# Shulk97/JPEG_detection_Resnet_SSD

Measured on AMD Instinct MI355X. Metric: images/sec (train) ResNet50-DCT-SSD300, higher is better.
Workload: dtype f32; 1 GPU; SSD300 ResNet50-DCT 'deconv' archi, 32 images/GPU, 300x300 JPEG-DCT inputs (Y 38x38x64 + chroma 19x19), fwd+loss+bwd+SGD(+RCCL all-reduce); batch and encoded targets resident in HBM: host->device upload, target encoding and the per-step loss read-back of fit_generator are outside the timed region (DESIGN.md section 6 has those rates); archi=deconv, global_batch=32, parallelism=dp1

## Files before the change

include/dj_hip.h:

```cpp
#ifndef DJ_HIP_H
#define DJ_HIP_H
#include <stddef.h>
#include <stdint.h>

#ifdef __cplusplus
extern "C" {
#endif

const char* dj_last_error(void);
#define DJ_ABI_VERSION 3
int dj_abi_version(void);

#define DJ_F32 0
#define DJ_F16 1
#define DJ_BF16 2

typedef struct dj_conv2d_desc {
  int batch;
  int in_h, in_w, in_c;
  int out_h, out_w, out_c;
  int kernel_h, kernel_w;
  int stride_h, stride_w;
  int dilation_h, dilation_w;
  int pad_top, pad_left;
// ... 25 lines not shown
int dj_conv2d_nhwc_dgrad_relumask(const dj_conv2d_desc* d, const float* dy, const float* w, const float* bias, float* dx,
                                  int beta, const float* mask_x, int ld_mask, void* stream);

int dj_conv2d_fwd_addrelu_supported(const dj_conv2d_desc* d);
int dj_conv2d_nhwc_fwd_addrelu(const dj_conv2d_desc* d, const float* x, const float* w, const float* bias, float* y,
                               const float* pro_scale, const float* pro_shift, const float* res, int ld_res,
                               const float* res_scale, const float* res_shift, float* sum_out, int ld_sum, int relu,
                               float* stats, void* stream);
int dj_conv2d_nhwc_fwd_addrelu_ws(const dj_conv2d_desc* d, const float* x, const float* w, const float* bias, float* y,
                                  const float* pro_scale, const float* pro_shift, const float* res, int ld_res,
                                  const float* res_scale, const float* res_shift, float* sum_out, int ld_sum, int relu,
                                  float* stats, float* workspace, long workspace_floats, void* stream);

#define DJ_BN_ACC_REPLICAS 16
typedef struct dj_bn_train {
  double* acc;
  unsigned* ticket;
  const float* gamma;
  const float* beta;
  float* moving_mean;
  float* moving_var;
  float* scale;
  float* shift;
  float* save_mean;
  float* save_invstd;
  float eps, momentum;
} dj_bn_train;
int dj_conv2d_nhwc_fwd_bn(const dj_conv2d_desc* d, const float* x, const float* w, const float* bias, float* y,
                          const float* pro_scale, const float* pro_shift, int pro_relu, const float* res, int ld_res,
                          const float* res_scale, const float* res_shift, float* sum_out, int ld_sum,
                          const dj_bn_train* bn, void* stream);

void dj_set_fast_path(int enable);

int dj_set_compute_mode(int mode);
int dj_set_thread_compute_mode(int mode);
int dj_get_compute_mode(void);

int dj_conv2d_tune_configs(void);
int dj_conv2d_tune_set(int dir, const dj_conv2d_desc* d, int cfg, int splits);
int dj_conv2d_default_config(int dir, const dj_conv2d_desc* d, int* cfg, int* splits);

int dj_conv2d_nhwc_wgrad(const dj_conv2d_desc* d, const float* x, const float* dy, float* dw,
                         const float* pro_scale, const float* pro_shift, int pro_relu, int dw_zeroed, void* stream);

int dj_conv2d_nhwc_fwd_t(const dj_conv2d_desc* d, const void* x, int dt_x, const void* w, int dt_w, const float* bias, void* y,
                         int dt_y, const float* pro_scale, const float* pro_shift, int pro_relu, int relu, float* stats,
                         const void* res, int ld_res, const float* res_scale, const float* res_shift, void* sum_out,
                         int ld_sum, int dt_sum, float* workspace, long workspace_floats, void* stream);
int dj_conv2d_nhwc_dgrad_t(const dj_conv2d_desc* d, const void* dy, int dt_dy, const void* w, int dt_w, const float* bias,
                           void* dx, int dt_dx, int beta, const void* z, int ld_z, int dt_z, const float* mean, const float* invstd,
                           const float* scale, const float* shift, float* partial, void* stream);
int dj_shadow_weights(const float* w, void* w16, void* wbf, long n, void* stream);
int dj_conv2d_nhwc_wgrad_t(const dj_conv2d_desc* d, const void* x, int dt_x, const void* dy, int dt_dy, float* dw,
                           const float* pro_scale, const float* pro_shift, int pro_relu, int dw_zeroed, void* stream);

int dj_reduce_rows(long rows);
int dj_colstats_partial(const float* x, long rows, int C, int ld, float* partial, void* stream);
int dj_colsum_partial(const float* dy, long rows, int C, int ld, float* partial, void* stream);
int dj_colreduce_finalize(const float* partial, int nrows, int C, int which, float* out, int beta, void* stream);
int dj_colsum_direct(const float* x, long rows, int C, int ld, float* out, int beta, void* stream);
#define DJ_COLSUM_PARTS 32
typedef struct dj_colsum_part {
  const float* x;
  float* out;
  long rows;
// ... 215 lines not shown
```

jpeg_detection_resnet_ssd_amd/_lib.py:

```python
import ctypes
import os
from ctypes import POINTER, Structure, c_char_p, c_double, c_float, c_int, c_long, c_void_p

_HERE = os.path.dirname(os.path.abspath(__file__))
LIB_PATH = os.environ.get("DJ_LIB_PATH") or os.path.join(_HERE, "csrc", "libdj_hip.so")


class DjError(RuntimeError):
    pass


class BnTrain(Structure):
    _fields_ = [("acc", c_void_p), ("ticket", c_void_p), ("gamma", c_void_p), ("beta", c_void_p),
                ("moving_mean", c_void_p), ("moving_var", c_void_p), ("scale", c_void_p), ("shift", c_void_p),
                ("save_mean", c_void_p), ("save_invstd", c_void_p), ("eps", c_float), ("momentum", c_float)]


class CopyPart(Structure):
    _fields_ = [("src", c_void_p), ("dst", c_void_p), ("ld_src", c_long), ("ld_dst", c_long), ("rows", c_long),
                ("cols", c_long), ("beta", c_int)]


class ColsumPart(Structure):
    _fields_ = [("x", c_void_p), ("out", c_void_p), ("rows", c_long), ("C", c_int), ("ld", c_int), ("beta", c_int)]
# ... 66 lines not shown
    "dj_conv2d_nhwc_fwd": (c_int, [POINTER(ConvDesc), FP, FP, FP, FP, FP, FP, c_int, c_int, FP, c_void_p]),
    "dj_conv2d_nhwc_fwd_ws": (c_int, [POINTER(ConvDesc), FP, FP, FP, FP, FP, FP, c_int, c_int, FP, FP, c_long, c_void_p]),
    "dj_conv2d_fwd_workspace_floats": (c_long, [POINTER(ConvDesc), c_int]),
    "dj_conv2d_nhwc_dgrad": (c_int, [POINTER(ConvDesc), FP, FP, FP, FP, c_int, c_void_p]),
    "dj_conv2d_nhwc_dgrad_bnbwd": (c_int, [POINTER(ConvDesc), FP, FP, FP, FP, c_int, FP, FP, FP, FP, FP, c_void_p]),
    "dj_conv2d_dgrad_relumask_supported": (c_int, [POINTER(ConvDesc)]),
    "dj_conv2d_nhwc_dgrad_relumask": (c_int, [POINTER(ConvDesc), FP, FP, FP, FP, c_int, FP, c_int, c_void_p]),
    "dj_conv2d_nhwc_wgrad": (c_int, [POINTER(ConvDesc), FP, FP, FP, FP, FP, c_int, c_int, c_void_p]),
    "dj_conv2d_nhwc_fwd_t": (c_int, [POINTER(ConvDesc), FP, c_int, FP, c_int, FP, FP, c_int, FP, FP, c_int, c_int, FP, FP, c_int, FP,
                                     FP, FP, c_int, c_int, FP, c_long, c_void_p]),
    "dj_conv2d_nhwc_dgrad_t": (c_int, [POINTER(ConvDesc), FP, c_int, FP, c_int, FP, FP, c_int, c_int, FP, c_int, c_int, FP, FP, FP,
                                       FP, FP, c_void_p]),
    "dj_shadow_weights": (c_int, [FP, FP, FP, c_long, c_void_p]),
    "dj_conv2d_nhwc_wgrad_t": (c_int, [POINTER(ConvDesc), FP, c_int, FP, c_int, FP, FP, FP, c_int, c_int, c_void_p]),
    "dj_affine_act_t": (c_int, [FP, c_int, c_int, FP, FP, FP, c_int, c_int, FP, FP, FP, c_int, c_int, c_long, c_int, c_int,
                                c_void_p]),
    "dj_bn_bwd_reduce_t": (c_int, [FP, c_int, c_int, FP, c_int, c_int, FP, c_int, c_int, FP, FP, FP, FP, c_int, c_long, c_int, FP,
                                   c_void_p]),
    "dj_bn_bwd_apply_t": (c_int, [FP, c_int, c_int, FP, c_int, c_int, FP, c_int, c_int, FP, FP, c_int, FP, FP, FP, FP, c_int,
                                  c_int, c_long, c_int, FP, c_int, c_int, c_int, c_void_p]),
    "dj_relu_bwd_t": (c_int, [FP, c_int, c_int, FP, c_int, c_int, FP, c_int, c_int, c_long, c_int, c_int, c_void_p]),
    "dj_copy2d_t": (c_int, [FP, c_int, c_long, FP, c_int, c_long, c_long, c_long, c_int, c_void_p]),
    "dj_conv2d_fwd_addrelu_supported": (c_int, [POINTER(ConvDesc)]),
    "dj_conv2d_nhwc_fwd_addrelu": (c_int, [POINTER(ConvDesc), FP, FP, FP, FP, FP, FP, FP, c_int, FP, FP, FP, c_int, c_int, FP,
                                           c_void_p]),
    "dj_conv2d_nhwc_fwd_addrelu_ws": (c_int, [POINTER(ConvDesc), FP, FP, FP, FP, FP, FP, FP, c_int, FP, FP, FP, c_int, c_int,
                                              FP, FP, c_long, c_void_p]),
    "dj_colsum_direct": (c_int, [FP, c_long, c_int, c_int, FP, c_int, c_void_p]),
    "dj_colsum_multi": (c_int, [POINTER(ColsumPart), c_int, c_void_p]),
    "dj_copy2d_multi": (c_int, [POINTER(CopyPart), c_int, c_void_p]),
    "dj_conv2d_nhwc_fwd_bn": (c_int, [POINTER(ConvDesc), FP, FP, FP, FP, FP, FP, c_int, FP, c_int, FP, FP, FP, c_int,
                                      POINTER(BnTrain), c_void_p]),
    "dj_set_fast_path": (None, [c_int]),
    "dj_set_compute_mode": (c_int, [c_int]),
    "dj_set_thread_compute_mode": (c_int, [c_int]),
    "dj_get_compute_mode": (c_int, []),
    "dj_conv2d_tune_configs": (c_int, []),
    "dj_conv2d_tune_set": (c_int, [c_int, POINTER(ConvDesc), c_int, c_int]),
    "dj_conv2d_default_config": (c_int, [c_int, POINTER(ConvDesc), POINTER(c_int), POINTER(c_int)]),
    "dj_reduce_rows": (c_int, [c_long]),
    "dj_colstats_partial": (c_int, [FP, c_long, c_int, c_int, FP, c_void_p]),
    "dj_colsum_partial": (c_int, [FP, c_long, c_int, c_int, FP, c_void_p]),
    "dj_colreduce_finalize": (c_int, [FP, c_int, c_int, c_int, FP, c_int, c_void_p]),
    "dj_bn_train_finalize": (c_int, [FP, c_int, c_long, FP, FP, FP, c_float, c_float, FP, FP, FP, FP, FP, FP, c_int,
                                     c_void_p]),
    "dj_bn_infer_coeffs": (c_int, [FP, FP, FP, FP, c_float, FP, FP, c_int, c_void_p]),
    "dj_affine_act": (c_int, [FP, c_int, FP, FP, FP, c_int, FP, FP, FP, c_int, c_long, c_int, c_int, c_void_p]),
    "dj_bn_bwd_reduce": (c_int, [FP, c_int, FP, c_int, FP, c_int, FP, FP, FP, FP, c_int, c_long, c_int, FP, c_void_p]),
    "dj_bn_bwd_finalize": (c_int, [FP, c_int, c_long, FP, FP, FP, FP, FP, FP, FP, FP, c_int, c_void_p]),
    "dj_bn_bwd_apply": (c_int, [FP, c_int, FP, c_int, FP, c_int, FP, FP, c_int, FP, FP, FP, FP, c_int, c_long, c_int,
                                FP, c_int, c_int, c_void_p]),
    "dj_relu_bwd": (c_int, [FP, c_int, FP, c_int, FP, c_int, c_long, c_int, c_int, c_void_p]),
    "dj_copy2d": (c_int, [FP, c_long, FP, c_long, c_long, c_long, c_int, c_void_p]),
    "dj_upsample2x": (c_int, [FP, c_int, FP, c_int, c_int, c_int, c_int, c_int, c_void_p]),
    "dj_l2norm_fwd": (c_int, [FP, c_int, FP, FP, c_int, FP, c_long, c_int, c_void_p]),
    "dj_l2norm_bwd": (c_int, [FP, c_int, FP, c_int, FP, FP, FP, c_int, FP, c_long, c_int, c_int, c_void_p]),
    "dj_maxpool2d_fwd": (c_int, [FP, FP] + [c_int] * 13 + [c_void_p, c_void_p]),
    "dj_maxpool2d_bwd": (c_int, [FP, FP, FP] + [c_int] * 14 + [c_void_p, c_void_p]),
    "dj_softmax_fwd": (c_int, [FP, FP, c_long, c_int, c_void_p]),
    "dj_softmax_bwd": (c_int, [FP, FP, c_long, FP, c_long, c_int, c_int, c_void_p]),
    "dj_ssd_loss_workspace_floats": (c_long, [c_long]),
    "dj_ssd_loss_fwd": (c_int, [FP, FP, c_long, c_int, c_int, c_int, c_float, FP, FP, c_void_p]),
    "dj_ssd_loss_bwd": (c_int, [FP, FP, c_long, c_int, c_float, c_float, FP, FP, FP, c_void_p]),
    "dj_categorical_crossentropy": (c_int, [FP, FP, c_long, c_int, c_float, FP, FP, FP, c_void_p]),
    "dj_sgd_momentum_update": (c_int, [FP, FP, FP, c_long, c_float, c_float, c_int, c_float, c_float, FP, c_void_p]),
    "dj_decode_detections_workspace_floats": (c_long, [c_int, c_int, c_int, c_int]),
# ... 73 lines not shown
```

jpeg_detection_resnet_ssd_amd/csrc/dj_conv.hip:

```cpp
#include "../../include/dj_hip.h"
#include "dj_conv_launch.h"
#include <string.h>
#include <map>
#include <mutex>
#include <atomic>
#include <array>
#include <algorithm>

static thread_local char g_err[512] = "";
void dj_set_error(const char* fmt, ...) {
  va_list ap;
  va_start(ap, fmt);
  vsnprintf(g_err, sizeof(g_err), fmt, ap);
  va_end(ap);
}
extern "C" const char* dj_last_error(void) { return g_err; }
extern "C" int dj_abi_version(void) { return DJ_ABI_VERSION; }

std::atomic<bool> g_dj_allow_fast{true};
extern "C" void dj_set_fast_path(int enable) { g_dj_allow_fast.store(enable != 0, std::memory_order_relaxed); }

static std::atomic<int> g_default_compute_mode{0};
static thread_local int tl_compute_mode = -1;
int dj_compute_mode() { return tl_compute_mode >= 0 ? tl_compute_mode : g_default_compute_mode.load(std::memory_order_relaxed); }
extern "C" int dj_set_compute_mode(int mode) {
  int prev = g_default_compute_mode.load(std::memory_order_relaxed);
  if (mode >= 0 && mode <= 5) g_default_compute_mode.store(mode, std::memory_order_relaxed);
  return prev;
}
extern "C" int dj_set_thread_compute_mode(int mode) {
  int prev = tl_compute_mode;
  if (mode >= -1 && mode <= 5) tl_compute_mode = mode;
  return prev;
}
extern "C" int dj_get_compute_mode(void) { return dj_compute_mode(); }

extern template int dj_launch_cfg<0, 0>(int, const DjIgemmParams&, int, hipStream_t);
extern template int dj_launch_cfg<0, 1>(int, const DjIgemmParams&, int, hipStream_t);
extern template int dj_launch_cfg<1, 1>(int, const DjIgemmParams&, int, hipStream_t);
extern template int dj_launch_cfg<2, 0>(int, const DjIgemmParams&, int, hipStream_t);

static int choose_cfg(long M, long N, long K, bool allow_split, int* splits_out) {
  int bn;
  if (N > 96) {
    long pad128 = (long)dj_cdiv(N, 128) * 128, pad64 = (long)dj_cdiv(N, 64) * 64;
    bn = (pad64 < pad128) ? 64 : 128;
  } else if (N > 32 && (long)dj_cdiv(N, 64) * 64 <= (long)dj_cdiv(N, 32) * 32) {
    bn = 64;
  } else {
    bn = 32;
  }
  int cfg;
  auto tiles = [&](int bm, int b_n) { return (long)dj_cdiv(M, bm) * dj_cdiv(N, b_n); };
// ... 791 lines not shown
```

jpeg_detection_resnet_ssd_amd/csrc/dj_conv_launch.h:

```cpp
#pragma once
#include "../../include/dj_hip.h"
#include "dj_igemm.h"
#include "dj_igemm_fast.h"
#include <stdlib.h>
#include <atomic>

struct TileCfg {
  int bm, bn;
};
static const TileCfg kCfgs[] = {{128, 128}, {128, 64}, {64, 64}, {128, 32}, {128, 128}, {128, 64}, {64, 64}, {64, 64}, {128, 64}, {128, 128}, {128, 64}, {64, 64}, {64, 64}, {128, 64}};
enum {
  CFG_128x128 = 0,
  CFG_128x64,
  CFG_64x64,
  CFG_128x32,
  CFG_128x128_S1,
  CFG_128x64_S1,
  CFG_64x64_S1,
  CFG_64x64_S1P,
  CFG_128x64_S1P,
  CFG_128x128_P,
  CFG_128x64_P,
  CFG_64x64_P,
  CFG_64x64_PK2,
// ... 83 lines not shown
      dj_set_error("residual-add prologue outside the forward GEMM");
      return DJ_ERR_ARG;
    }
  }
  if (p.mask_x) {
    if constexpr (AM == 1 && BMD == 1) {
      static std::atomic<bool> done2{false};
      return launch_kernel(dj_igemm_kernel<BM, BN, WM, WN, AM, BMD, 2>, Cfg::SMEM_BYTES, BM, BN, p, splits, s, &done2);
    } else {
      dj_set_error("masked accumulate outside the input-gradient GEMM");
      return DJ_ERR_ARG;
    }
  }
  return launch_kernel(dj_igemm_kernel<BM, BN, WM, WN, AM, BMD>, Cfg::SMEM_BYTES, BM, BN, p, splits, s, &done[0]);
}

template <int BM, int BN, int AM, int BMD>
static int launch_k2(const DjIgemmParams& p, int splits, hipStream_t s, int fast) {
  using Cfg = DjIgemmCfg<BM, BN, 2, 2, AM, BMD>;
  if (fast == 1)
    return launch_fast<BM, BN, 2, 2, AM, BMD, 0, 4, 0, 2, 0>(2 * Cfg::SMEM_BYTES, p, splits, s, 512);
  if (fast == 3) {
    if constexpr (AM == 0 && BMD == 0) {
      return launch_fast<BM, BN, 2, 2, AM, BMD, 3, 4, 0, 2, 0>(2 * Cfg::SMEM_BYTES, p, splits, s, 512);
    } else {
      dj_set_error("residual-add prologue outside the forward GEMM");
      return DJ_ERR_ARG;
    }
  }
  return launch_fast<BM, BN, 2, 2, AM, BMD, 1, 4, 0, 2, 0>(2 * Cfg::SMEM_BYTES, p, splits, s, 512);
}

extern std::atomic<bool> g_dj_allow_fast;

int dj_compute_mode();

template <int AM, int BMD>
static int fast_mode(const DjIgemmParams& p) {
  if (!g_dj_allow_fast.load(std::memory_order_relaxed) || !p.vecA || !p.vecB) return 0;
  if (p.a_bytes <= 0 || p.b_bytes <= 0) return 0;
  if (AM != 2 && p.srcC % 32 != 0) return 0;
  if (AM != 2 && p.M >= (1 << 22)) return 0;
  if (AM == 1 && (p.sH != 1 || p.sW != 1)) return 0;
  if (AM == 2 && (p.srcC % 4 != 0 || p.K >= (1 << 24))) return 0;
  if (BMD == 0 && (p.N % 4 != 0 || p.ldb % 4 != 0)) return 0;
  if (BMD == 1 && p.srcC % 32 != 0) return 0;
  if (p.A2) return (AM == 0 && BMD == 0 && p.pro_scale) ? 3 : 0;
  return p.pro_scale ? 2 : 1;
}

static inline int dj_fast_mode_fwd(const DjIgemmParams& p) { return fast_mode<0, 0>(p); }

template <int AM, int BMD>
int dj_launch_lowp(int cfg, const DjIgemmParams& p, int splits, hipStream_t s, int fast, int mode);

template <int AM, int BMD>
int dj_launch_cfg(int cfg, const DjIgemmParams& p, int splits, hipStream_t s) {
  const int fast = fast_mode<AM, BMD>(p);
  int mode = dj_compute_mode();
  if (mode == 5) mode = 0;
  if (cfg >= N_CFG) {
    cfg -= N_CFG;
    if (fast && mode == 0 && cfg < N_CFG) return dj_launch_lowp<AM, BMD>(cfg, p, splits, s, fast, 4);
  }
  if (fast && mode != 0 && cfg >= 0 && cfg < N_CFG) {
    return dj_launch_lowp<AM, BMD>(cfg, p, splits, s, fast, mode);
// ... 41 lines not shown
```

jpeg_detection_resnet_ssd_amd/csrc/dj_conv_launch_h16.h:

```cpp
#pragma once
#include "dj_conv_launch.h"
#include "dj_igemm_h16.h"

template <int BM, int BN, int AM, int BMD, int PRO, int PREC, int BK, int PF, int AT, int BT, int NP>
static int launch_h16_np(int smem_bytes, const DjIgemmParams& p, int splits, hipStream_t s) {
  if constexpr (AM == 1 && BMD == 1 && PRO == 0) {
    if (p.bnb_z) {
      static std::atomic<bool> done1{false};
      return launch_kernel(dj_igemm_h16_kernel<BM, BN, AM, BMD, PRO, PREC, BK, PF, 1, AT, BT, NP>, smem_bytes, BM, BN, p, splits,
                           s, &done1, 256);
    }
    if constexpr (PREC >= 3 && AT == 0 && BT == 0) {
      if (p.mask_x) {
        static std::atomic<bool> done2{false};
        return launch_kernel(dj_igemm_h16_kernel<BM, BN, AM, BMD, PRO, PREC, BK, PF, 2, AT, BT, NP>, smem_bytes, BM, BN, p,
                             splits, s, &done2, 256);
      }
    }
  }
  if (p.mask_x) {
    dj_set_error("masked accumulate: no such kernel for this GEMM role / arithmetic mode");
    return DJ_ERR_ARG;
  }
  static std::atomic<bool> done0{false};
  return launch_kernel(dj_igemm_h16_kernel<BM, BN, AM, BMD, PRO, PREC, BK, PF, 0, AT, BT, NP>, smem_bytes, BM, BN, p, splits, s,
                       &done0, 256);
}

template <int BM, int BN, int AM, int BMD, int PRO, int PREC, int BK, int PF, int AT, int BT>
static int launch_h16_kernel(int smem_bytes, const DjIgemmParams& p, int splits, hipStream_t s) {
  if constexpr (PRO != 3) {
    static const bool np_off = getenv("DJ_NO_NP") != nullptr;
    const bool same_grid = (AM != 2) || (p.sH == 1 && p.sW == 1 && p.rowH == p.srcH && p.rowW == p.srcW);
    if (!np_off && p.KH == 1 && p.KW == 1 && p.pT == 0 && p.pL == 0 && same_grid)
      return launch_h16_np<BM, BN, AM, BMD, PRO, PREC, BK, PF, AT, BT, 1>(smem_bytes, p, splits, s);
  }
  return launch_h16_np<BM, BN, AM, BMD, PRO, PREC, BK, PF, AT, BT, 0>(smem_bytes, p, splits, s);
}

template <int BM, int BN, int AM, int BMD, int PREC, int BK, int PF, int AT, int BT>
static int launch_h16(const DjIgemmParams& p, int splits, hipStream_t s, int fast) {
  constexpr int SMEM_BYTES = DjH16Cfg<BM, BN, AM, BMD, BK>::SMEM_BYTES * (PREC == 4 ? 3 : PREC == 3 ? 2 : 1);
  static_assert(SMEM_BYTES <= 160 * 1024, "LDS of a CU");
  if (fast == 3) {
    if constexpr (AM == 0 && BMD == 0) {
      return launch_h16_kernel<BM, BN, AM, BMD, 3, PREC, BK, PF, AT, BT>(SMEM_BYTES, p, splits, s);
    } else {
      dj_set_error("residual-add prologue outside the forward GEMM");
      return DJ_ERR_ARG;
    }
  }
  if (fast == 1)
    return launch_h16_kernel<BM, BN, AM, BMD, 0, PREC, BK, PF, AT, BT>(SMEM_BYTES, p, splits, s);
  if constexpr (AM != 1) {
    return launch_h16_kernel<BM, BN, AM, BMD, 1, PREC, BK, PF, AT, BT>(SMEM_BYTES, p, splits, s);
  } else {
    dj_set_error("prologue on the input-gradient GEMM");
    return DJ_ERR_ARG;
  }
}

template <int BM, int BN, int AM, int BMD, int PREC, int PF, int AT, int BT>
static int launch_h16_depth(const DjIgemmParams& p, int splits, hipStream_t s, int fast, bool deep) {
  static const bool bk32 = getenv("DJ_H16_BK32") != nullptr;
  if constexpr (PREC >= 3 && BM == 128) {
    if (deep && !bk32 && p.srcC % 16 == 0 && p.kchunk % 16 == 0)
      return launch_h16<BM, BN, AM, BMD, PREC, 16, PF, AT, BT>(p, splits, s, fast);
  } else if constexpr (AM != 2) {
// ... 59 lines not shown
```

jpeg_detection_resnet_ssd_amd/csrc/dj_igemm_h16.h:

```cpp
#pragma once
#include "dj_igemm.h"
#include "dj_igemm_fast.h"

typedef short dj_tr4 __attribute__((__vector_size__(4 * sizeof(short))));
typedef short dj_s16x8 __attribute__((ext_vector_type(8)));
typedef _Float16 dj_half8 __attribute__((ext_vector_type(8)));
typedef __bf16 dj_bf16x8 __attribute__((ext_vector_type(8)));
typedef short __attribute__((address_space(3))) dj_lds_short;
typedef unsigned int u32x2 __attribute__((ext_vector_type(2)));

template <int DT>
struct DjRaw {
  using type = f32x4;
};
template <>
struct DjRaw<1> {
  using type = u32x2;
};
template <>
struct DjRaw<2> {
  using type = u32x2;
};

template <int DT>
__device__ __forceinline__ typename DjRaw<DT>::type dj_buf_ldraw(__amdgpu_buffer_rsrc_t r, unsigned off) {
  if constexpr (DT == 0) {
    return dj_buf_ld4(r, off);
  } else {
    return __builtin_bit_cast(u32x2, __builtin_amdgcn_raw_buffer_load_b64(r, (int)off, 0, 0));
  }
}

template <int DT>
__device__ __forceinline__ f32x4 dj_raw_to_f32(typename DjRaw<DT>::type v) {
  if constexpr (DT == 0) {
// ... 24 lines not shown
template <int PREC>
__device__ __forceinline__ dj_short4 dj_round4(f32x4 v) {
  if (PREC == 1) return __builtin_bit_cast(dj_short4, dj_to_half4(v));
  return dj_to_bf16x4(v);
}

__device__ __forceinline__ void dj_split_store(short* dst, f32x4 v, int lo_off) {
  const dj_short4 hi = dj_to_bf16x4(v);
  const f32x4 back = {__builtin_bit_cast(float, (unsigned)(unsigned short)hi.x << 16),
                      __builtin_bit_cast(float, (unsigned)(unsigned short)hi.y << 16),
                      __builtin_bit_cast(float, (unsigned)(unsigned short)hi.z << 16),
                      __builtin_bit_cast(float, (unsigned)(unsigned short)hi.w << 16)};
  *reinterpret_cast<dj_short4*>(dst) = hi;
  *reinterpret_cast<dj_short4*>(dst + lo_off) = dj_to_bf16x4(v - back);
}

__device__ __forceinline__ f32x4 dj_bf16x4_to_f32(dj_short4 h) {
  return f32x4{__builtin_bit_cast(float, (unsigned)(unsigned short)h.x << 16), __builtin_bit_cast(float, (unsigned)(unsigned short)h.y << 16),
               __builtin_bit_cast(float, (unsigned)(unsigned short)h.z << 16), __builtin_bit_cast(float, (unsigned)(unsigned short)h.w << 16)};
}
__device__ __forceinline__ void dj_split_store3(short* dst, f32x4 v, int lo_off) {
  const dj_short4 hi = dj_to_bf16x4(v);
  const f32x4 r1 = v - dj_bf16x4_to_f32(hi);
  const dj_short4 mid = dj_to_bf16x4(r1);
  const f32x4 r2 = r1 - dj_bf16x4_to_f32(mid);
  *reinterpret_cast<dj_short4*>(dst) = hi;
  *reinterpret_cast<dj_short4*>(dst + lo_off) = mid;
  *reinterpret_cast<dj_short4*>(dst + 2 * lo_off) = dj_to_bf16x4(r2);
}

template <int BM, int BN, int AM, int BMD, int PRO, int PREC, int BK = 32, int PF = 1, int EPI = 0, int AT = 0, int BT = 0, int NP = 0>
__global__ __launch_bounds__(256) void dj_igemm_h16_kernel(const DjIgemmParams p) {
  static_assert(NP == 0 || PRO != 3, "NP: not with the residual-add prologue (which keeps row indices of its own)");
  static_assert(EPI == 0 || (AM == 1 && BMD == 1), "BatchNormalization backward statistics: input-gradient GEMM only");
  static_assert(EPI != 2 || (PRO == 0 && AT == 0 && BT == 0), "masked accumulate: fp32 tensors, no prologue");
  static_assert(PREC < 3 || (AT == 0 && BT == 0), "float32x3 / float32x6: fp32 tensors");
  constexpr int EA = AT ? 2 : 4, EB = BT ? 2 : 4;
  using ARaw = typename DjRaw<AT>::type;
  using BRaw = typename DjRaw<BT>::type;
  constexpr bool A_COPY = (AT == PREC) && PRO == 0 && PREC < 3, B_COPY = (BT == PREC) && PREC < 3;
  using Cfg = DjH16Cfg<BM, BN, AM, BMD, BK>;
  constexpr int IMGS = (PREC == 4) ? 3 : (PREC == 3) ? 2 : 1;
  constexpr int STAGE = Cfg::STAGE_H * IMGS;
  constexpr int TM = Cfg::TM, TN = Cfg::TN, NA = Cfg::NA, NB = Cfg::NB;
  constexpr int PA = Cfg::PA, PB = Cfg::PB, KCH = Cfg::KCH, RPP = Cfg::RPP;
  constexpr int WN = 2;
  extern __shared__ __attribute__((aligned(16))) float smem_base[];
  short* const smem = reinterpret_cast<short*>(smem_base);

  const int tid = threadIdx.x;
  const int lane = tid & 63, wave = tid >> 6;
  const int wm = wave / WN, wn = wave % WN;
  const int l31 = lane & 31, lh = lane >> 5;

  const int tiles_n = (p.N + BN - 1) / BN;
  int tile_id, ky;
  dj_tile_of_workgroup(tile_id, ky);
  const int tile_m = tile_id / tiles_n;
  const int tile_n = tile_id - tile_m * tiles_n;
  const int m0 = tile_m * BM, n0 = tile_n * BN;
  const int kbeg = ky * p.kchunk;
  const int kend = min(p.K, kbeg + p.kchunk);
  const int nk = (kend - kbeg + BK - 1) / BK;

  const __amdgpu_buffer_rsrc_t rA = __builtin_amdgcn_make_buffer_rsrc((void*)p.A, 0, p.a_bytes, 0x00020000);
  const __amdgpu_buffer_rsrc_t rB = __builtin_amdgcn_make_buffer_rsrc((void*)p.B, 0, p.b_bytes, 0x00020000);
// ... 28 lines not shown
    for (int j = 0; j < NA; ++j) {
      int m = m0 + ar0 + ARPP * j;
      if (m < p.M) {
        int img, h, w;
        dj_row_decompose(p, m, img, h, w);
        int rh = (AM == 0) ? h * p.sH - p.pT : h + p.pT;
        int rw = (AM == 0) ? w * p.sW - p.pL : w + p.pL;
        a_rh[j] = rh;
        a_rw[j] = rw;
        a_off[j] = ((img * p.srcH * p.srcW + rh * p.srcW + rw) * p.ldsrc + 4 * ac) * EA;
        row_valid |= 1u << j;
      } else {
        a_rh[j] = -(1 << 28);
        a_rw[j] = -(1 << 28);
        a_off[j] = NP ? (int)0x80000000 : 0;
      }
    }
  } else {
#pragma unroll
    for (int i = 0; i < NA; ++i) {
      int mm = m0 + 4 * (ac + ACG * i);
      a2_ok[i] = mm < p.M;
      int tap = mm / p.srcC;
      a2_c[i] = mm - tap * p.srcC;
      int kh = tap / p.KW;
      int kw = tap - kh * p.KW;
      a2_dh[i] = kh * p.dH - p.pT;
      a2_dw[i] = kw * p.dW - p.pL;
      if (PRO) {
        a2_sc[i] = dj_buf_ld4(rS, a2_ok[i] ? (unsigned)a2_c[i] * 4u : DJ_OOB);
        a2_sh[i] = dj_buf_ld4(rT, a2_ok[i] ? (unsigned)a2_c[i] * 4u : DJ_OOB);
      }
      row_valid |= a2_ok[i] ? (1u << i) : 0u;
      if (NP) a2_c[i] = a2_ok[i] ? a2_c[i] * EA : (int)0x80000000;
    }
  }
  int np_row = (NP && AM == 2) ? (kbeg + ar0) * p.ldsrc * EA : 0;
  const int np_step = BK * p.ldsrc * EA;
  int b_off[NB];
  bool b_ok[NB];
  if (BMD == 0) {
    int n = n0 + 4 * bcn;
#pragma unroll
    for (int j = 0; j < NB; ++j) {
      b_ok[j] = n < p.N;
      b_off[j] = ((bkr0 + BKSTEP * j) * p.ldb + n) * EB;
    }
  } else {
#pragma unroll
    for (int j = 0; j < NB; ++j) {
      int n = n0 + br0 + RPP * j;
      b_ok[j] = n < p.N;
      b_off[j] = (n * p.ldb + 4 * bc) * EB;
    }
  }

  int t_c0 = 0, t_kh = 0, t_kw = 0, t_tap = 0;
  if (AM != 2 || BMD == 1) {
    t_tap = kbeg / p.srcC;
    t_c0 = kbeg - t_tap * p.srcC;
    t_kh = t_tap / p.KW;
    t_kw = t_tap - t_kh * p.KW;
  }

  struct Regs {
    ARaw ra[NA];
    BRaw rb[NB];
    unsigned a_valid;
    f32x4 psc, psh;
    ARaw ra2[PRO == 3 ? NA : 1];
    f32x4 psc2, psh2;
    int pro_c0;
  };
  Regs r0, r1;
  r0.a_valid = r1.a_valid = 0;
  r0.pro_c0 = r1.pro_c0 = 0;
  r0.psc = r1.psc = r0.psc2 = r1.psc2 = f32x4{1.f, 1.f, 1.f, 1.f};
  r0.psh = r1.psh = r0.psh2 = r1.psh2 = f32x4{0.f, 0.f, 0.f, 0.f};

  auto issue_loads = [&](Regs& R, int kcur, bool live) {
    ARaw(&ra)[NA] = R.ra;
    BRaw(&rb)[NB] = R.rb;
    ARaw(&ra2)[PRO == 3 ? NA : 1] = R.ra2;
    unsigned& a_valid = R.a_valid;
    f32x4 &psc = R.psc, &psh = R.psh, &psc2 = R.psc2, &psh2 = R.psh2;
    int& pro_c0 = R.pro_c0;
    if (AM != 2) {
      const int dh = t_kh * p.dH, dw = t_kw * p.dW;
      const int delta = (AM == 0) ? ((dh * p.srcW + dw) * p.ldsrc + t_c0) * EA : (-(dh * p.srcW + dw) * p.ldsrc + t_c0) * EA;
      if (PRO == 1) {
        psc = dj_buf_ld4(rS, (unsigned)(t_c0 + 4 * ac) * 4u);
        psh = dj_buf_ld4(rT, (unsigned)(t_c0 + 4 * ac) * 4u);
      }
      if (PRO == 3) {
        pro_c0 = t_c0;
        psc = dj_ld4(p.pro_scale + (t_c0 + 4 * ac));
        psh = dj_ld4(p.pro_shift + (t_c0 + 4 * ac));
        psc2 = f32x4{1.f, 1.f, 1.f, 1.f};
        psh2 = f32x4{0.f, 0.f, 0.f, 0.f};
        if (p.pro_scale2) {
          psc2 = dj_ld4(p.pro_scale2 + (t_c0 + 4 * ac));
          psh2 = dj_ld4(p.pro_shift2 + (t_c0 + 4 * ac));
        }
      }
      a_valid = 0;
      if (PRO == 3) {
        const unsigned cb = (unsigned)(4 * ac + t_c0);
#pragma unroll
        for (int j = 0; j < NA; ++j) {
          const bool ok = live && pm[j] >= 0;
          const unsigned m = (unsigned)pm[j];
          ra[j] = dj_buf_ldraw<AT>(rA, ok ? (__umul24(m, (unsigned)p.ldsrc) + cb) * (unsigned)EA : DJ_OOB);
          ra2[j] = dj_buf_ldraw<AT>(rA2, ok ? (__umul24(m, (unsigned)p.ldsrc2) + cb) * (unsigned)EA : DJ_OOB);
          a_valid |= ok ? (1u << j) : 0u;
        }
      } else if (NP) {
        a_valid = row_valid;
        const int udelta = live ? delta : (int)0x80000000;
#pragma unroll
        for (int j = 0; j < NA; ++j) ra[j] = dj_buf_ldraw<AT>(rA, (unsigned)(a_off[j] + udelta));
      } else {
#pragma unroll
      for (int j = 0; j < NA; ++j) {
        int h = (AM == 0) ? a_rh[j] + dh : a_rh[j] - dh;
        int w = (AM == 0) ? a_rw[j] + dw : a_rw[j] - dw;
        bool ok = live && (unsigned)h < (unsigned)p.srcH && (unsigned)w < (unsigned)p.srcW;
        ra[j] = dj_buf_ldraw<AT>(rA, ok ? (unsigned)(a_off[j] + delta) : DJ_OOB);
        a_valid |= ok ? (1u << j) : 0u;
      }
      }
    } else if (NP) {
      a_valid = row_valid;
      const int urow = live ? np_row : (int)0x80000000;
#pragma unroll
      for (int i = 0; i < NA; ++i) ra[i] = dj_buf_ldraw<AT>(rA, (unsigned)(urow + a2_c[i]));
      np_row += np_step;
    } else {
      a_valid = 0;
      const int kp = kcur + ar0;
      const int hw = p.rowH * p.rowW;
      int img = (int)((float)kp * p.inv_rowHW);
      int rem = kp - img * hw;
      int adj = (rem < 0) ? -1 : ((rem >= hw) ? 1 : 0);
      img += adj;
      rem -= adj * hw;
      int oh = (int)((float)rem * p.inv_rowW);
      int ow = rem - oh * p.rowW;
      int adj2 = (ow < 0) ? -1 : ((ow >= p.rowW) ? 1 : 0);
      oh += adj2;
      ow -= adj2 * p.rowW;
      const bool rowok = live && kp < kend;
      const int h0 = oh * p.sH, w0 = ow * p.sW, pb = img * p.srcH * p.srcW;
#pragma unroll
      for (int i = 0; i < NA; ++i) {
        int h = h0 + a2_dh[i], w = w0 + a2_dw[i];
        bool ok = rowok && a2_ok[i] && (unsigned)h < (unsigned)p.srcH && (unsigned)w < (unsigned)p.srcW;
        unsigned off = (unsigned)((pb + h * p.srcW + w) * p.ldsrc + a2_c[i]) * (unsigned)EA;
        ra[i] = dj_buf_ldraw<AT>(rA, ok ? off : DJ_OOB);
        a_valid |= ok ? (1u << i) : 0u;
      }
    }
    if (BMD == 0) {
      const int base = kcur * p.ldb * EB;
#pragma unroll
      for (int j = 0; j < NB; ++j) {
        bool ok = live && b_ok[j] && (AM != 2 || kcur + bkr0 + BKSTEP * j < kend);
        rb[j] = dj_buf_ldraw<BT>(rB, ok ? (unsigned)(b_off[j] + base) : DJ_OOB);
      }
    } else {
      const unsigned base = (unsigned)(t_tap * p.bTapStride + t_c0) * (unsigned)EB;
#pragma unroll
      for (int j = 0; j < NB; ++j) rb[j] = dj_buf_ldraw<BT>(rB, (live && b_ok[j]) ? (unsigned)b_off[j] + base : DJ_OOB);
    }
    if (AM != 2 || BMD == 1) {
      t_c0 += BK;
      const int wrap = (t_c0 >= p.srcC) ? 1 : 0;
      t_c0 = wrap ? 0 : t_c0;
      t_tap += wrap;
      t_kw += wrap;
      const int wrap2 = (t_kw >= p.KW) ? 1 : 0;
      t_kw = wrap2 ? 0 : t_kw;
      t_kh += wrap2;
    }
  };

  auto store_a = [&](const Regs& R, short* sA, int j) {
    const ARaw(&ra)[NA] = R.ra;
    const ARaw(&ra2)[PRO == 3 ? NA : 1] = R.ra2;
    const unsigned a_valid = R.a_valid;
    const f32x4 psc = R.psc, psh = R.psh, psc2 = R.psc2, psh2 = R.psh2;
    const int pro_c0 = R.pro_c0;
    {
      short* dst = (AM != 2) ? sA + (ar0 + ARPP * j) * PA + 4 * ac : sA + ar0 * PA + 4 * (ac + ACG * j);
      if constexpr (A_COPY) {
        *reinterpret_cast<u32x2*>(dst) = ra[j];
        return;
      }
      f32x4 v = dj_raw_to_f32<AT>(ra[j]);
      if (PRO) {
        f32x4 sc = (AM == 2) ? a2_sc[j] : psc, sh = (AM == 2) ? a2_sh[j] : psh;
        v = v * sc + sh;
        if (PRO == 3) v += dj_raw_to_f32<AT>(ra2[j]) * psc2 + psh2;
        bool ok = (NP && AM == 2) ? true : (bool)((a_valid >> j) & 1u);
        const float lo = ok ? relu_floor : 0.f, hi = ok ? INFINITY : 0.f;
        v.x = __builtin_amdgcn_fmed3f(v.x, lo, hi);
        v.y = __builtin_amdgcn_fmed3f(v.y, lo, hi);
        v.z = __builtin_amdgcn_fmed3f(v.z, lo, hi);
        v.w = __builtin_amdgcn_fmed3f(v.w, lo, hi);
        if (PRO == 3 && store_sum) {
          const unsigned e = __umul24((unsigned)pm[j], (unsigned)p.ld_sum) + (unsigned)(4 * ac + pro_c0);
          if (p.sum_dt == 0)
            __builtin_amdgcn_raw_buffer_store_b128(__builtin_bit_cast(u32x4, v), rY, ok ? (int)(e * 4u) : (int)DJ_OOB, 0, 0);
          else
            __builtin_amdgcn_raw_buffer_store_b64(__builtin_bit_cast(u32x2, p.sum_dt == 1 ? dj_round4<1>(v) : dj_round4<2>(v)),
                                                  rY, ok ? (int)(e * 2u) : (int)DJ_OOB, 0, 0);
        }
      }
      if constexpr (PREC == 4) {
        dj_split_store3(dst, v, Cfg::STAGE_H);
      } else if constexpr (PREC == 3) {
        dj_split_store(dst, v, Cfg::STAGE_H);
      } else {
        *reinterpret_cast<dj_short4*>(dst) = dj_round4<PREC>(v);
      }
    }
  };
  auto store_b = [&](const Regs& R, short* sB, int j) {
    const BRaw(&rb)[NB] = R.rb;
    {
      short* dst = (BMD == 0) ? sB + (bkr0 + BKSTEP * j) * PB + 4 * bcn : sB + (br0 + RPP * j) * PB + 4 * bc;
      if constexpr (B_COPY)
        *reinterpret_cast<u32x2*>(dst) = rb[j];
      else if constexpr (PREC == 4)
        dj_split_store3(dst, dj_raw_to_f32<BT>(rb[j]), Cfg::STAGE_H);
      else if constexpr (PREC == 3)
        dj_split_store(dst, dj_raw_to_f32<BT>(rb[j]), Cfg::STAGE_H);
// ... 129 lines not shown
```

Before: 1605 images/sec.

## Add per-tap offset cache and incremental pixel walk for gathered GEMM operands

Adds two new A-operand gather variants to the h16 implicit-GEMM kernel, enabled by default for fp32 split-precision modes. For the forward and data-gradient paths, per-row address offsets and validity are recomputed only when the filter tap changes. For the weight gradient, the gathered operand advances an incremental (image, row, col) pixel walker instead of re-dividing the k index every step. Both aim to cut per-iteration integer and address arithmetic in the load loop, at the cost of extra registers and more template instantiations.

```diff
diff --git a/include/dj_hip.h b/include/dj_hip.h
--- a/include/dj_hip.h
+++ b/include/dj_hip.h
@@ -81,6 +81,8 @@
                           const dj_bn_train* bn, void* stream);
 
 void dj_set_fast_path(int enable);
+
+void dj_set_gather_variants(int enable);
 
 int dj_set_compute_mode(int mode);
 int dj_set_thread_compute_mode(int mode);
diff --git a/jpeg_detection_resnet_ssd_amd/_lib.py b/jpeg_detection_resnet_ssd_amd/_lib.py
--- a/jpeg_detection_resnet_ssd_amd/_lib.py
+++ b/jpeg_detection_resnet_ssd_amd/_lib.py
@@ -122,6 +122,7 @@
     "dj_conv2d_nhwc_fwd_bn": (c_int, [POINTER(ConvDesc), FP, FP, FP, FP, FP, FP, c_int, FP, c_int, FP, FP, FP, c_int,
                                       POINTER(BnTrain), c_void_p]),
     "dj_set_fast_path": (None, [c_int]),
+    "dj_set_gather_variants": (None, [c_int]),
     "dj_set_compute_mode": (c_int, [c_int]),
     "dj_set_thread_compute_mode": (c_int, [c_int]),
     "dj_get_compute_mode": (c_int, []),
diff --git a/jpeg_detection_resnet_ssd_amd/csrc/dj_conv.hip b/jpeg_detection_resnet_ssd_amd/csrc/dj_conv.hip
--- a/jpeg_detection_resnet_ssd_amd/csrc/dj_conv.hip
+++ b/jpeg_detection_resnet_ssd_amd/csrc/dj_conv.hip
@@ -19,6 +19,8 @@
 
 std::atomic<bool> g_dj_allow_fast{true};
 extern "C" void dj_set_fast_path(int enable) { g_dj_allow_fast.store(enable != 0, std::memory_order_relaxed); }
+std::atomic<bool> g_dj_gather_variants{true};
+extern "C" void dj_set_gather_variants(int enable) { g_dj_gather_variants.store(enable != 0, std::memory_order_relaxed); }
 
 static std::atomic<int> g_default_compute_mode{0};
 static thread_local int tl_compute_mode = -1;
diff --git a/jpeg_detection_resnet_ssd_amd/csrc/dj_conv_launch.h b/jpeg_detection_resnet_ssd_amd/csrc/dj_conv_launch.h
--- a/jpeg_detection_resnet_ssd_amd/csrc/dj_conv_launch.h
+++ b/jpeg_detection_resnet_ssd_amd/csrc/dj_conv_launch.h
@@ -139,6 +139,7 @@
 }
 
 extern std::atomic<bool> g_dj_allow_fast;
+extern std::atomic<bool> g_dj_gather_variants;
 
 int dj_compute_mode();
 
diff --git a/jpeg_detection_resnet_ssd_amd/csrc/dj_conv_launch_h16.h b/jpeg_detection_resnet_ssd_amd/csrc/dj_conv_launch_h16.h
--- a/jpeg_detection_resnet_ssd_amd/csrc/dj_conv_launch_h16.h
+++ b/jpeg_detection_resnet_ssd_amd/csrc/dj_conv_launch_h16.h
@@ -34,6 +34,19 @@
     const bool same_grid = (AM != 2) || (p.sH == 1 && p.sW == 1 && p.rowH == p.srcH && p.rowW == p.srcW);
     if (!np_off && p.KH == 1 && p.KW == 1 && p.pT == 0 && p.pL == 0 && same_grid)
       return launch_h16_np<BM, BN, AM, BMD, PRO, PREC, BK, PF, AT, BT, 1>(smem_bytes, p, splits, s);
+  }
+  if constexpr (PRO != 3 && PREC >= 3) {
+    static const bool np_off = getenv("DJ_NO_NP") != nullptr;
+    if (!np_off && g_dj_gather_variants.load(std::memory_order_relaxed)) {
+      if constexpr (AM == 2) {
+        static const bool walk_off = getenv("DJ_NO_WALK") != nullptr;
+        if (!walk_off && p.srcC % BM == 0)
+          return launch_h16_np<BM, BN, AM, BMD, PRO, PREC, BK, PF, AT, BT, 3>(smem_bytes, p, splits, s);
+      } else {
+        static const bool ht_off = getenv("DJ_NO_TAPCACHE") != nullptr;
+        if (!ht_off) return launch_h16_np<BM, BN, AM, BMD, PRO, PREC, BK, PF, AT, BT, 2>(smem_bytes, p, splits, s);
+      }
+    }
   }
   return launch_h16_np<BM, BN, AM, BMD, PRO, PREC, BK, PF, AT, BT, 0>(smem_bytes, p, splits, s);
 }
diff --git a/jpeg_detection_resnet_ssd_amd/csrc/dj_igemm_h16.h b/jpeg_detection_resnet_ssd_amd/csrc/dj_igemm_h16.h
--- a/jpeg_detection_resnet_ssd_amd/csrc/dj_igemm_h16.h
+++ b/jpeg_detection_resnet_ssd_amd/csrc/dj_igemm_h16.h
@@ -1,6 +1,7 @@
 #pragma once
 #include "dj_igemm.h"
 #include "dj_igemm_fast.h"
+#include "dj_walk.h"
 
 typedef short dj_tr4 __attribute__((__vector_size__(4 * sizeof(short))));
 typedef short dj_s16x8 __attribute__((ext_vector_type(8)));
@@ -91,6 +92,8 @@
 template <int BM, int BN, int AM, int BMD, int PRO, int PREC, int BK = 32, int PF = 1, int EPI = 0, int AT = 0, int BT = 0, int NP = 0>
 __global__ __launch_bounds__(256) void dj_igemm_h16_kernel(const DjIgemmParams p) {
   static_assert(NP == 0 || PRO != 3, "NP: not with the residual-add prologue (which keeps row indices of its own)");
+  static_assert(NP != 2 || AM != 2, "NP 2 (per-tap offsets) is for the k-contiguous A operand");
+  static_assert(NP != 3 || AM == 2, "NP 3 (pixel walk) is for the weight gradient's gathered operand");
   static_assert(EPI == 0 || (AM == 1 && BMD == 1), "BatchNormalization backward statistics: input-gradient GEMM only");
   static_assert(EPI != 2 || (PRO == 0 && AT == 0 && BT == 0), "masked accumulate: fp32 tensors, no prologue");
   static_assert(PREC < 3 || (AT == 0 && BT == 0), "float32x3 / float32x6: fp32 tensors");
@@ -185,11 +188,23 @@
         a2_sh[i] = dj_buf_ld4(rT, a2_ok[i] ? (unsigned)a2_c[i] * 4u : DJ_OOB);
       }
       row_valid |= a2_ok[i] ? (1u << i) : 0u;
-      if (NP) a2_c[i] = a2_ok[i] ? a2_c[i] * EA : (int)0x80000000;
-    }
-  }
-  int np_row = (NP && AM == 2) ? (kbeg + ar0) * p.ldsrc * EA : 0;
+      if (NP == 1) a2_c[i] = a2_ok[i] ? a2_c[i] * EA : (int)0x80000000;
+    }
+  }
+  int np_row = (NP == 1 && AM == 2) ? (kbeg + ar0) * p.ldsrc * EA : 0;
   const int np_step = BK * p.ldsrc * EA;
+  const DjWalkGeom walk_g{p.rowH, p.rowW, p.srcH, p.srcW, p.sH, p.sW, p.ldsrc * EA};
+  DjWalkStep walk_s{};
+  DjWalkPos walk{};
+  int walk_dh = 0, walk_dw = 0;
+  if (NP == 3) {
+    const int tap = m0 / p.srcC, cb = m0 - tap * p.srcC;
+    const int kh = tap / p.KW, kw = tap - kh * p.KW;
+    walk_dh = kh * p.dH - p.pT;
+    walk_dw = kw * p.dW - p.pL;
+    walk_s = dj_walk_step(walk_g, BK);
+    walk = dj_walk_init(walk_g, kbeg + ar0, walk_dh, walk_dw, (cb + 4 * ac) * EA);
+  }
   int b_off[NB];
   bool b_ok[NB];
   if (BMD == 0) {
@@ -215,6 +230,25 @@
     t_kh = t_tap / p.KW;
     t_kw = t_tap - t_kh * p.KW;
   }
+
+  int a_tap[NP == 2 ? NA : 1];
+  unsigned tap_valid = 0;
+  auto recompute_tap = [&]() {
+    if (NP == 2) {
+      const int dh = t_kh * p.dH, dw = t_kw * p.dW;
+      const int tapdelta = (AM == 0) ? (dh * p.srcW + dw) * p.ldsrc * EA : -(dh * p.srcW + dw) * p.ldsrc * EA;
+      tap_valid = 0;
+#pragma unroll
+      for (int j = 0; j < NA; ++j) {
+        const int h = (AM == 0) ? a_rh[j] + dh : a_rh[j] - dh;
+        const int w = (AM == 0) ? a_rw[j] + dw : a_rw[j] - dw;
+        const bool ok = ((unsigned)h < (unsigned)p.srcH) & ((unsigned)w < (unsigned)p.srcW);
+        a_tap[j] = ok ? a_off[j] + tapdelta : (int)0x80000000;
+        tap_valid |= ok ? (1u << j) : 0u;
+      }
+    }
+  };
+  recompute_tap();
 
   struct Regs {
     ARaw ra[NA];
@@ -267,6 +301,11 @@
           ra2[j] = dj_buf_ldraw<AT>(rA2, ok ? (__umul24(m, (unsigned)p.ldsrc2) + cb) * (unsigned)EA : DJ_OOB);
           a_valid |= ok ? (1u << j) : 0u;
         }
+      } else if (NP == 2) {
+        a_valid = tap_valid;
+        const unsigned uc = live ? (unsigned)(t_c0 * EA) : 0x80000000u;
+#pragma unroll
+        for (int j = 0; j < NA; ++j) ra[j] = dj_buf_ldraw<AT>(rA, (unsigned)a_tap[j] + uc);
       } else if (NP) {
         a_valid = row_valid;
         const int udelta = live ? delta : (int)0x80000000;
@@ -282,6 +321,14 @@
         a_valid |= ok ? (1u << j) : 0u;
       }
       }
+    } else if (NP == 3) {
+      const int ih = __mul24(walk.oh, p.sH) + walk_dh, iw = __mul24(walk.ow, p.sW) + walk_dw;
+      const bool ok = live & dj_walk_inside(walk_g, walk, ih, iw, kend);
+      const unsigned voff = ok ? (unsigned)walk.off : 0x80000000u;
+      a_valid = ok ? 0xFFFFFFFFu : 0u;
+#pragma unroll
+      for (int i = 0; i < NA; ++i) ra[i] = dj_buf_ldraw<AT>(rA, voff + (unsigned)(4 * ACG * EA * i));
+      dj_walk_advance(walk_g, walk_s, walk);
     } else if (NP) {
       a_valid = row_valid;
       const int urow = live ? np_row : (int)0x80000000;
@@ -334,6 +381,7 @@
       const int wrap2 = (t_kw >= p.KW) ? 1 : 0;
       t_kw = wrap2 ? 0 : t_kw;
       t_kh += wrap2;
+      if (NP == 2 && wrap) recompute_tap();
     }
   };
 
@@ -354,7 +402,7 @@
         f32x4 sc = (AM == 2) ? a2_sc[j] : psc, sh = (AM == 2) ? a2_sh[j] : psh;
         v = v * sc + sh;
         if (PRO == 3) v += dj_raw_to_f32<AT>(ra2[j]) * psc2 + psh2;
-        bool ok = (NP && AM == 2) ? true : (bool)((a_valid >> j) & 1u);
+        bool ok = (NP == 1 && AM == 2) ? true : (bool)((a_valid >> j) & 1u);
         const float lo = ok ? relu_floor : 0.f, hi = ok ? INFINITY : 0.f;
         v.x = __builtin_amdgcn_fmed3f(v.x, lo, hi);
         v.y = __builtin_amdgcn_fmed3f(v.y, lo, hi);
diff --git a/jpeg_detection_resnet_ssd_amd/csrc/dj_walk.h b/jpeg_detection_resnet_ssd_amd/csrc/dj_walk.h
--- /dev/null
+++ b/jpeg_detection_resnet_ssd_amd/csrc/dj_walk.h
@@ -0,0 +1,62 @@
+#pragma once
+
+#if defined(__HIPCC__) || defined(__CUDACC__)
+#define DJ_WALK_HD __host__ __device__ __forceinline__
+#else
+#define DJ_WALK_HD inline
+#endif
+
+struct DjWalkGeom {
+  int rowH, rowW, srcH, srcW, sH, sW, pix_bytes;
+};
+
+struct DjWalkStep {
+  int step;
+  int sw, sh;
+  int c0, c1, c2;
+};
+
+struct DjWalkPos {
+  int ow, oh;
+  int kp;
+  int off;
+};
+
+DJ_WALK_HD DjWalkStep dj_walk_step(const DjWalkGeom& g, int step) {
+  DjWalkStep s;
+  const int hw = g.rowH * g.rowW;
+  const int s_img = step / hw, r = step - s_img * hw;
+  s.step = step;
+  s.sh = r / g.rowW;
+  s.sw = r - s.sh * g.rowW;
+  s.c0 = ((s_img * g.srcH + s.sh * g.sH) * g.srcW + s.sw * g.sW) * g.pix_bytes;
+  s.c1 = (g.sH * g.srcW - g.rowW * g.sW) * g.pix_bytes;
+  s.c2 = (g.srcH - g.rowH * g.sH) * g.srcW * g.pix_bytes;
+  return s;
+}
+
+DJ_WALK_HD DjWalkPos dj_walk_init(const DjWalkGeom& g, int kp, int dh, int dw, int base) {
+  DjWalkPos w;
+  const int hw = g.rowH * g.rowW;
+  const int img = kp / hw, rem = kp - img * hw;
+  w.kp = kp;
+  w.oh = rem / g.rowW;
+  w.ow = rem - w.oh * g.rowW;
+  w.off = ((img * g.srcH + w.oh * g.sH + dh) * g.srcW + w.ow * g.sW + dw) * g.pix_bytes + base;
+  return w;
+}
+
+DJ_WALK_HD bool dj_walk_inside(const DjWalkGeom& g, const DjWalkPos& w, int ih, int iw, int kend) {
+  return (w.kp < kend) & ((unsigned)ih < (unsigned)g.srcH) & ((unsigned)iw < (unsigned)g.srcW);
+}
+
+DJ_WALK_HD void dj_walk_advance(const DjWalkGeom& g, const DjWalkStep& s, DjWalkPos& w) {
+  w.kp += s.step;
+  w.ow += s.sw;
+  const bool c1 = w.ow >= g.rowW;
+  w.ow -= c1 ? g.rowW : 0;
+  w.oh += s.sh + (c1 ? 1 : 0);
+  const bool c2 = w.oh >= g.rowH;
+  w.oh -= c2 ? g.rowH : 0;
+  w.off += s.c0 + (c1 ? s.c1 : 0) + (c2 ? s.c2 : 0);
+}
```

New measurement: 1631 images/sec, median of 6. 1.6% higher.
